# syl051088/DynaAlign

Measured on AMD Instinct MI355X. Metric: sequence-pairs/sec (MinHash k=4 n_hash=500; NW BLOSUM62) at 1/2/4/8 MI355X, higher is better.
Workload: dtype u32

## Files before the change

### dynaalign_amd/csrc/api.cpp

```cpp
#include <sched.h>

#include <algorithm>
#include <atomic>
#include <chrono>
#include <climits>
#include <cmath>
#include <condition_variable>
#include <cstddef>
#include <map>
#include <memory>
#include <cstdlib>
#include <cstring>
#include <functional>
#include <mutex>
#include <random>
#include <string>
#include <thread>
#include <vector>

#include "da_common.hpp"

namespace da { size_t destroy_cached_comms(); }

namespace da {
// ... 326 lines not shown
  return rows;
}
int64_t rows_per_block(int64_t n, size_t bytes_per_elem) { return std::min(block_rows(n, bytes_per_elem), n); }

}
}

using namespace da;

namespace da {
namespace {
bool env_flag(const char *name) { return getenv(name) != nullptr; }
int64_t env_i64(const char *name, int64_t dflt) { const char *e = getenv(name); return e ? atoll(e) : dflt; }
uint64_t env_u64(const char *name, uint64_t dflt) { const char *e = getenv(name); return e ? strtoull(e, nullptr, 10) : dflt; }
enum MhExpand { MH_EXPAND_DEFAULT, MH_EXPAND_ROWS, MH_EXPAND_ROWSPIPE, MH_EXPAND_PIPE, MH_EXPAND_TILES };
Config parse_config() {
  Config c;
  c.mh_no_dedup = env_flag("DYNAALIGN_MH_NO_DEDUP");
  c.mh_no_sparse = env_flag("DYNAALIGN_MH_NO_SPARSE");
  c.mh_no_pipe = env_flag("DYNAALIGN_MH_NO_PIPE");
  c.mh_pipe_one_stream = env_flag("DYNAALIGN_MH_PIPE_ONE_STREAM");
  c.mh_dedup_min_n = env_i64("DYNAALIGN_MH_DEDUP_MIN_N", -1);
  c.mh_dedup_max_pct = env_i64("DYNAALIGN_MH_DEDUP_MAX_PCT", -1);
  c.mh_sparse_max_pairs = std::min<uint64_t>(env_u64("DYNAALIGN_MH_SPARSE_MAX_PAIRS", 400000000ull), 0xfffffff0ull);
  c.mh_no_hybrid = env_flag("DYNAALIGN_MH_NO_HYBRID");
  c.mh_hybrid_min_n = env_i64("DYNAALIGN_MH_HYBRID_MIN_N", -1);
  c.mh_hybrid_dedup = env_flag("DYNAALIGN_MH_HYBRID_DEDUP");
  if (const char *e = getenv("DYNAALIGN_MH_EXPAND"))
    c.mh_expand = !strcmp(e, "rows") ? MH_EXPAND_ROWS : !strcmp(e, "rowspipe") ? MH_EXPAND_ROWSPIPE : !strcmp(e, "pipe") ? MH_EXPAND_PIPE
                : !strcmp(e, "tiles") ? MH_EXPAND_TILES : MH_EXPAND_DEFAULT;
  c.mh_pipe_step = (int)std::max<int64_t>(0, env_i64("DYNAALIGN_MH_PIPE_STEP", 0));
  c.mh_pipe_wg = (int)std::max<int64_t>(0, std::min<int64_t>(4, env_i64("DYNAALIGN_MH_PIPE_WG", 0)));
  c.mh_pipe_head = (int)std::max<int64_t>(0, env_i64("DYNAALIGN_MH_PIPE_HEAD", 0));
  const int pb = (int)env_i64("DYNAALIGN_PLANE_BITS", 0);
  c.plane_bits = (pb == 32 || pb == 16 || pb == 15 || pb == 14 || pb == 12) ? pb : 0;
  c.k2_no_asm = env_flag("DYNAALIGN_K2_NO_ASM");
  c.k2_persist = env_flag("DYNAALIGN_K2_PERSIST");
  c.k2_wg_per_cu = (int)std::max<int64_t>(0, env_i64("DYNAALIGN_K2_WG_PER_CU", 0));
  c.nw_no_dedup = env_flag("DYNAALIGN_NW_NO_DEDUP");
  c.nw_int32 = env_flag("DYNAALIGN_NW_INT32");
  c.nw_no_prefix = env_flag("DYNAALIGN_NW_NO_PREFIX_SHARE");
  c.nw_dedup_min_n = env_i64("DYNAALIGN_NW_DEDUP_MIN_N", -1);
  c.no_host_widen = env_flag("DYNAALIGN_NO_HOST_WIDEN");
  c.plain_d2h = env_flag("DYNAALIGN_PLAIN_D2H");
  c.no_buffer_cache = env_flag("DYNAALIGN_NO_BUFFER_CACHE");
  c.d2h_threads = (int)std::max<int64_t>(0, env_i64("DYNAALIGN_D2H_THREADS", 0));
  c.buffer_cache_pct = (int)std::max<int64_t>(0, std::min<int64_t>(90, env_i64("DYNAALIGN_BUFFER_CACHE_PCT", 30)));
  c.block_bytes = env_u64("DYNAALIGN_BLOCK_BYTES", 0);
  c.trace = env_flag("DYNAALIGN_TRACE");
  c.louvain_debug = env_flag("DYNAALIGN_LOUVAIN_DEBUG");
  c.louvain_threads = (int)std::max<int64_t>(0, env_i64("DYNAALIGN_LOUVAIN_THREADS", 0));
  return c;
}
std::atomic<const Config *> g_config{nullptr};
}
const Config &config() {
  const Config *c = g_config.load(std::memory_order_acquire);
  if (!c) {
    const Config *fresh = new Config(parse_config());
    if (g_config.compare_exchange_strong(c, fresh, std::memory_order_acq_rel)) c = fresh;
    else delete fresh;
  }
  return *c;
}
}
extern "C" void da_config_reload(void) { da::g_config.store(new da::Config(da::parse_config()), std::memory_order_release); }
// ... 371 lines not shown
  const hipStream_t stream = k.stream;
  int rc;
  const bool two = expand_stream_packed(k.n_hash);
  const int wg = cfg.mh_pipe_wg > 0 ? cfg.mh_pipe_wg : two ? 2 : 1, head = cfg.mh_pipe_head > 0 ? cfg.mh_pipe_head : two ? 1 : 4,
            step = cfg.mh_pipe_step > 0 ? cfg.mh_pipe_step : two ? 8 : 4;
  const bool alt = !cfg.mh_pipe_one_stream;
  std::vector<int64_t> cuts{0};
  while (cuts.back() < KB) cuts.push_back(std::min(KB, cuts.back() + (cuts.size() == 1 ? head : step)));
  const size_t C = cuts.size() - 1;
  const PipeLease lease(3 * C + 2);
  PipeRes *const pr = lease.r;
  if (!pr) return MH_NO_PIPE;
  hipEvent_t *pe = pr->ev.data();
  DA_HIP_TRY(hipStreamWaitEvent(pr->side, k.ev[2], 0));
  if ((rc = launch_mh_compare_edges_u16(c.planes.as<uint32_t>(), U, k.n_hash, k.dtab, k.ld_d, stream, c.bits, k.pk)) != DA_OK) return rc;
  if ((rc = launch_expand_stream_lists(k.d.p.uidx, k.n, U, k.ex, stream)) != DA_OK) return rc;
  DA_HIP_TRY(hipEventRecord(pe[3 * C], stream));
  if (c.split()) {
    if ((rc = c.lists(stream)) != DA_OK) return rc;
    DA_HIP_TRY(hipEventRecord(pe[3 * C + 1], stream));
  }
  if (alt) { DA_HIP_TRY(hipStreamWaitEvent(pr->alt[0], pe[3 * C], 0)); DA_HIP_TRY(hipStreamWaitEvent(pr->alt[1], pe[3 * C], 0)); }
  for (size_t ci = 0; ci < C; ++ci) {
    if ((rc = launch_mh_compare_bands_u16(c.planes.as<uint32_t>(), U, k.n_hash, k.dtab, k.ld_d, cuts[ci], cuts[ci + 1], ci == 0 ? 4 : wg, pr->side, c.bits,
                                          k.pk)) != DA_OK) return rc;
    if (c.split()) {
      if (ci == 0) { DA_HIP_TRY(hipStreamWaitEvent(pr->side, pe[3 * C], 0)); DA_HIP_TRY(hipStreamWaitEvent(pr->side, pe[3 * C + 1], 0)); }
      if ((rc = c.fixup(DA_OUT_COMPACT, k.dtab, k.ld_d, pr->side, cuts[ci] * 8, cuts[ci + 1] * 8)) != DA_OK) return rc;
    }
    DA_HIP_TRY(hipEventRecord(pe[3 * ci], pr->side));
    const hipStream_t es = alt ? pr->alt[ci & 1] : stream;
    DA_HIP_TRY(hipStreamWaitEvent(es, pe[3 * ci], 0));
    DA_HIP_TRY(hipEventRecord(pe[3 * ci + 1], es));
    if ((rc = launch_expand_stream_rows(k.dtab, k.ld_d, k.d.p.uidx, k.n, U, k.n_hash, k.out, k.ld, k.ex, cuts[ci] * 1024, cuts[ci + 1] * 1024, es,
                                        (int)ci, k.pk)) != DA_OK) return rc;
    DA_HIP_TRY(hipEventRecord(pe[3 * ci + 2], es));
  }
  if (alt) for (size_t ci = (C >= 2 ? C - 2 : 0); ci < C; ++ci) DA_HIP_TRY(hipStreamWaitEvent(stream, pe[3 * ci + 2], 0));
  if ((rc = mh_finish(k, 5, MH_ROWS_PIPE, 2)) != DA_OK) return rc;
  k.route.chunks = k.route.expand_launches = (int)C;
  MhEvents::ms(k.route, 2, k.ev[2], pe[3 * (C - 1)]);
  MhEvents::ms(k.route, 3, k.ev[2], pe[3 * C]);
  LaunchUnion expand{k.ev[2]};
  for (size_t ci = 0; ci < C; ++ci) expand.add(pe[3 * ci + 1], pe[3 * ci + 2]);
  k.route.ms[4] = expand.total;
  return DA_OK;
}
static int mh_tiles_pipe(const MhCall &k) {
  const Config &cfg = da::config();
  const MhCodes &c = k.c;
  uint16_t *ftab = static_cast<uint16_t *>(k.ex);
  const hipStream_t stream = k.stream;
  const std::vector<int32_t> &ub = k.d.ub;
  const int64_t U = k.d.U, KB = mh_sym_bands(U), NB = (int64_t)ub.size() - 1, ld_f = ceil_div(k.n, 8) * 8;
  int rc;
  const int step = cfg.mh_pipe_step > 0 ? cfg.mh_pipe_step : 4, wg = cfg.mh_pipe_wg > 0 ? cfg.mh_pipe_wg : 2;
  const bool alt = !cfg.mh_pipe_one_stream;
  struct Chunk { int64_t kb0, kb1, ob0, ob1; };
  std::vector<Chunk> chunks;
  for (int64_t kb = 0, ob = 0; kb < KB;) {
    const int64_t kb1 = std::min(KB, kb + (chunks.empty() ? 1 : step));
    int64_t ob1 = ob;
    if (kb1 == KB) ob1 = NB;
    else while (ob1 < NB && (int64_t)ub[(size_t)ob1 + 1] <= kb1 * 1024) ++ob1;
    chunks.push_back({kb, kb1, ob, ob1});
    kb = kb1; ob = ob1;
  }
  const size_t C = chunks.size();
// ... 2941 lines not shown
```

### dynaalign_amd/csrc/da_common.hpp

```cpp
#pragma once

#include <hip/hip_runtime.h>

#include <cstdarg>
#include <cstdint>
#include <cstdio>
#include <string>

#include "../../include/dynaalign.h"

namespace da {
struct Config {
  bool mh_no_dedup = false, mh_no_sparse = false, mh_no_pipe = false, mh_pipe_one_stream = false;
  int64_t mh_dedup_min_n = -1, mh_dedup_max_pct = -1;
  uint64_t mh_sparse_max_pairs = 400000000ull;
  bool mh_no_hybrid = false, mh_hybrid_dedup = false;
  int64_t mh_hybrid_min_n = -1;
  int mh_expand = 0;
  int mh_pipe_step = 0, mh_pipe_wg = 0, mh_pipe_head = 0;
  int plane_bits = 0;
  bool k2_no_asm = false, k2_persist = false;
  int k2_wg_per_cu = 0;
  bool nw_no_dedup = false, nw_int32 = false, nw_no_prefix = false;
  int64_t nw_dedup_min_n = -1;
  bool no_host_widen = false, plain_d2h = false, no_buffer_cache = false;
  int d2h_threads = 0, buffer_cache_pct = 30;
  uint64_t block_bytes = 0;
  bool trace = false, louvain_debug = false;
  int louvain_threads = 0;
};
const Config &config();


std::string &last_error_ref();
int fail(int code, const char *fmt, ...) __attribute__((format(printf, 2, 3)));

#define DA_HIP_TRY(expr)                                                              \
  do {                                                                                \
    hipError_t _e = (expr);                                                           \
    if (_e != hipSuccess)                                                             \
      return ::da::fail(_e == hipErrorNoDevice || _e == hipErrorInvalidDevice         \
                            ? DA_ERR_NO_DEVICE                                        \
                            : DA_ERR_HIP,                                             \
                        "%s failed: %s (%s:%d)", #expr, hipGetErrorString(_e),        \
                        __FILE__, __LINE__);                                          \
  } while (0)

inline int64_t ceil_div(int64_t a, int64_t b) { return (a + b - 1) / b; }
inline int block_shape_ok(int64_t rows, int64_t n) {
  if (rows > 0x7fffffffLL || n > 0x7ffffff0LL) return fail(DA_ERR_UNSUPPORTED, "key block too large for one launch");
  return DA_OK;
}
// ... 120 lines not shown
                   nullptr, nullptr, nullptr, c0, c1);
}
size_t nw_sort_unique_workspace_bytes(int64_t n);
int launch_nw_sort_unique(const uint8_t *d_codes, const int64_t *d_off, int64_t n, void *d_work, size_t work_bytes, const int32_t **perm_out,
                          const uint8_t **lcp_out, hipStream_t stream);
struct NwDedupPlan {
  uint32_t *table; uint32_t table_size;
  int32_t *rep, *mult, *last, *fm, *fs, *pm, *ps, *uid_of, *uidx, *ufirst, *ulast, *ulen, *minfirst, *maxlast;
  int64_t *uoff;
  uint8_t *ucodes;
  size_t bytes;
};
NwDedupPlan nw_dedup_layout(void *work, int64_t n, int64_t total);
size_t nw_dedup_workspace_bytes(int64_t n, int64_t total);
int launch_nw_dedup_count(const uint8_t *d_codes, const int64_t *d_off, int64_t n, const NwDedupPlan &p, hipStream_t stream);
int launch_nw_dedup_build(const uint8_t *d_codes, const int64_t *d_off, int64_t n, int64_t U, const NwDedupPlan &p, hipStream_t stream,
                          bool first_order = false);
int launch_expand_unique(const uint16_t *d_D, int64_t ld_d, const int32_t *d_uidx, int64_t n, int kind, bool is_nw, int n_hash,
                         void *d_out, int64_t ld, hipStream_t stream, int nw_max_len = 0, uint16_t *d_F = nullptr,
                         const int32_t *d_ufirst = nullptr, int64_t U = 0, hipEvent_t after_gather = nullptr, hipEvent_t after_rows = nullptr,
                         int table_world = 1, int64_t table_rows_local = 0,
                         bool only_leftover = false);
bool expand_stream_ok(int64_t n, int64_t U, int n_hash, const void *d_out, int64_t ld);
size_t expand_stream_scratch_bytes(int64_t n, int64_t U);
bool expand_stream_packed(int n_hash);
int launch_expand_stream(const uint16_t *d_D, int64_t ld_d, const int32_t *d_uidx, int64_t n, int64_t U, int n_hash, double *d_out, int64_t ld,
                         void *d_scratch, hipStream_t stream, hipEvent_t after_lists = nullptr, bool pk = false);
int launch_expand_stream_lists(const int32_t *d_uidx, int64_t n, int64_t U, void *d_scratch, hipStream_t stream);
bool expand_stream_rect_ok(int64_t m, int64_t n, int64_t U_x, int64_t U_y, int n_hash, const void *d_out, int64_t ld);
int launch_expand_stream_rect(const uint16_t *d_D, int64_t ld_d, const int32_t *d_uidx_x, int64_t m, int64_t U_x, const int32_t *d_uidx_y, int64_t n,
                              int64_t U_y, int n_hash, double *d_out, int64_t ld, void *d_scratch, hipStream_t stream,
                              hipEvent_t after_lists = nullptr);
int launch_expand_stream_rows(const uint16_t *d_D, int64_t ld_d, const int32_t *d_uidx, int64_t n, int64_t U, int n_hash, double *d_out, int64_t ld,
                              void *d_scratch, int64_t row_begin, int64_t row_end, hipStream_t stream, int launch_no,
                              bool pk = false);
int launch_expand_rows(const uint16_t *d_F, int64_t ld_f, const int32_t *d_uidx, int64_t n, bool is_nw, int n_hash, int nw_max_len,
                       double *d_out, int64_t ld, int64_t band_begin, int64_t band_end, hipStream_t stream);
size_t expand_rows_workspace_bytes(int64_t n, int64_t U, int kind, bool is_nw, int n_hash, int nw_max_len);
int launch_upper_histogram(const uint16_t *d_m, int64_t ld, int64_t n, int nbins, unsigned long long *d_hist,
                           hipStream_t stream, int rank = 0, int world = 0, const int32_t *d_rowmap = nullptr);
int launch_extract_edges(const uint16_t *d_m, int64_t ld, int64_t n, const uint8_t *d_keep, int nbins,
                         bool include_diagonal, int32_t *d_i, int32_t *d_j, uint16_t *d_v, int64_t capacity,
                         unsigned long long *d_count, hipStream_t stream, int rank = 0, int world = 0,
                         const int32_t *d_rowmap = nullptr);
int launch_gather_columns(const uint16_t *d_D, int64_t ld_d, const int32_t *d_uidx, const int32_t *d_ufirst, int64_t n, int64_t U,
                          uint16_t *d_F, int64_t ld_f, bool from_first_tile, hipStream_t stream, int table_world = 1,
                          int64_t table_rows_local = 0, int64_t row_begin = 0, int64_t row_end = -1);
size_t edges_to_csr_workspace_bytes(int64_t m, int64_t n);
int launch_edges_to_csr(const int32_t *d_i, const int32_t *d_j, const uint16_t *d_v, int64_t m, int64_t n, void *d_work, size_t work_bytes,
                        int64_t *d_ptr, int32_t *d_adj, uint16_t *d_codes, uint16_t *d_loops, hipStream_t stream);
size_t knn_edges_workspace_bytes(int64_t n, int top);
int launch_knn_edges(const int32_t *d_idx, const uint16_t *d_key, int64_t ld, int64_t n, int top, bool mutual, bool is_nw, const uint16_t *d_self_key,
                     int self_code, bool loops, void *d_work, size_t work_bytes, int32_t *d_i, int32_t *d_j, uint16_t *d_v, uint64_t *d_count,
                     hipStream_t stream);
constexpr int DA_TOPK_MAX = 1024;
int launch_topk_rows(const uint16_t *d_keys, int64_t rows, int64_t n, int64_t ld, const uint16_t *d_rank, int rank_bits, int top, int32_t *d_idx,
                     int64_t ld_idx, uint16_t *d_key_out, int64_t ld_key, hipStream_t stream);
int launch_topk_rows_self(const uint16_t *d_keys, int64_t rows, int64_t n, int64_t ld, const uint16_t *d_rank, int rank_bits, int top, int64_t self_col0,
                          int32_t *d_idx, int64_t ld_idx, uint16_t *d_key_out, int64_t ld_key, uint16_t *d_self_key, hipStream_t stream);
int launch_topk_ranks(const uint32_t *d_keys, int64_t rows, int64_t n, int64_t ld, int64_t nbins, int top, int32_t *d_idx, int64_t ld_idx,
                      uint32_t *d_key_out, int64_t ld_key, hipStream_t stream);
int launch_topk_ranks_self(const uint32_t *d_keys, int64_t rows, int64_t n, int64_t ld, int64_t nbins, int top, int64_t self_col0, int32_t *d_idx,
                           int64_t ld_idx, uint32_t *d_key_out, int64_t ld_key, uint32_t *d_self_key, hipStream_t stream);
int launch_topk_values(const uint16_t *d_key, int64_t ld_key, int64_t rows, int top, int n_hash, double *d_val, int64_t ld_val, hipStream_t stream);
size_t threshold_rows_workspace_bytes(int64_t rows);
int launch_rect_histogram(const uint16_t *d_keys, int64_t rows, int64_t n, int64_t ld, int nbins, unsigned long long *d_hist, hipStream_t stream);
int launch_threshold_rows_count(const uint16_t *d_keys, int64_t rows, int64_t n, int64_t ld, const uint8_t *d_keep, int nbins, int64_t *d_rowptr,
// ... 37 lines not shown
```

### dynaalign_amd/csrc/minhash_kernels.hip

```cpp
#include "da_common.hpp"

#include <algorithm>
#include <atomic>
#include <mutex>
#include <vector>
#include <type_traits>

namespace da {
namespace {

__device__ __forceinline__ uint32_t rotl32(uint32_t v, int r) {
  return __builtin_rotateleft32(v, r);
}
__device__ __forceinline__ uint32_t mm3_scramble(uint32_t w) {
  w *= 0xcc9e2d51u;
  w = rotl32(w, 15);
  w *= 0x1b873593u;
  return w;
}
__device__ __forceinline__ uint32_t mm3_mix(uint32_t h, uint32_t kk) {
  h ^= kk;
  return rotl32(h, 13) * 5u + 0xe6546b64u;
}
__device__ __forceinline__ uint32_t mm3_final(uint32_t h, uint32_t len) {
// ... 1620 lines not shown
  double *tab = reinterpret_cast<double *>(er_lds + 128 * ER_STRIDE);
  const int64_t L = tile_begin + (int64_t)(blockIdx.x & 7) * per_xcd + (blockIdx.x >> 3);
  if (L >= ntiles || L >= tile_begin + (int64_t)((blockIdx.x & 7) + 1) * per_xcd) return;
  const TileId tt = decode_tile(L, T128, T128, true);
  if (!tt.valid || !expand_fast_takes(tt.ti, tt.tj, n, ld, out)) return;
  const int tid = threadIdx.x, wave = tid >> 6, lane = tid & 63;
  const int tx = ((wave & 1) << 3) + (lane & 7), ty = ((wave >> 1) << 3) + (lane >> 3);
  const int64_t I0 = (int64_t)tt.ti * 128, J0 = (int64_t)tt.tj * 128;
  uint4 st[8];
#pragma unroll
  for (int q = 0; q < 8; ++q) {
    const int row = (tid >> 4) + 16 * q;
    st[q] = *(reinterpret_cast<const uint4 *>(F + (int64_t)uidx[I0 + row] * ld_f + J0) + (tid & 15));
  }
  if (IS_NW) {
    for (int e = tid; e < tab_entries; e += 256) {
      const int mt = e / tab_stride, ln = e - mt * tab_stride;
      tab[e] = ln == 0 ? __longlong_as_double(0xFFF8000000000000ULL) : (double)mt / (double)ln;
    }
  } else {
    for (int e = tid; e < tab_entries; e += 256) tab[e] = (double)e / (double)n_hash;
  }
#pragma unroll
  for (int q = 0; q < 8; ++q)
    *reinterpret_cast<uint4 *>(er_lds + ((tid >> 4) + 16 * q) * ER_STRIDE + (tid & 15) * 16) = st[q];
  __syncthreads();
  auto widen = [&](uint32_t x) -> double {
    if (IS_NW) return tab[(x >> 8) * (uint32_t)tab_stride + (x & 255u)];
    return tab[x];
  };
  er_store_tile(er_lds, widen, out, ld, I0, J0, tx, ty);
}

constexpr int ES_THREADS = 1024, ES_COPIES = 4, ES_TICKETS = 128;
__global__ __launch_bounds__(256) void k_es_count(const int32_t *__restrict__ uidx, int n, uint32_t *__restrict__ cnt) {
  const int i = blockIdx.x * 256 + threadIdx.x;
  if (i < n) atomicAdd(&cnt[uidx[i]], 1u);
}
__global__ __launch_bounds__(1024) void k_es_scan(const uint32_t *__restrict__ cnt, int U, uint32_t *__restrict__ cstart, uint32_t *__restrict__ istart) {
  __shared__ uint64_t wsum[16];
  __shared__ uint64_t carry_s;
  const int tid = threadIdx.x, lane = tid & 63, wave = tid >> 6;
  if (tid == 0) carry_s = 0;
  __syncthreads();
  for (int base = 0; base < U; base += 1024) {
    const int u = base + tid;
    const uint32_t c = u < U ? cnt[u] : 0u;
    const uint64_t v = (uint64_t)c | ((uint64_t)((c + ES_COPIES - 1) / ES_COPIES) << 32);
    uint64_t x = v;
#pragma unroll
    for (int d = 1; d < 64; d <<= 1) {
      const uint64_t y = __shfl_up(x, d, 64);
      if (lane >= d) x += y;
    }
    if (lane == 63) wsum[wave] = x;
    __syncthreads();
    uint64_t woff = 0;
    for (int w = 0; w < wave; ++w) woff += wsum[w];
    const uint64_t carry = carry_s;
    if (u < U) {
      const uint64_t e = carry + woff + x - v;
      cstart[u] = (uint32_t)e;
      istart[u] = (uint32_t)(e >> 32);
    }
    __syncthreads();
    if (tid == 1023) carry_s = carry + woff + x;
    __syncthreads();
  }
  if (tid == 0) { cstart[U] = (uint32_t)carry_s; istart[U] = (uint32_t)(carry_s >> 32); }
}
__global__ __launch_bounds__(256) void k_es_fill(const int32_t *__restrict__ uidx, int n, int U, const uint32_t *__restrict__ cstart,
                                                 const uint32_t *__restrict__ istart, uint32_t *__restrict__ cursor, int32_t *__restrict__ cpos,
                                                 int2 *__restrict__ items) {
  const int i = blockIdx.x * 256 + threadIdx.x;
  if (i < n) {
    const int u = uidx[i];
    cpos[cstart[u] + atomicAdd(&cursor[u], 1u)] = i;
  }
  if (i < U) {
    const uint32_t first = istart[i], cnt = istart[i + 1] - first;
    for (uint32_t q = 0; q < cnt; ++q) items[first + q] = make_int2(i, (int)(q * ES_COPIES));
  }
}
__device__ __forceinline__ double es_ratio(uint32_t c, double dn, double rcp) {
  const double dc = (double)c, q0 = __dmul_rn(dc, rcp), e = __fma_rn(-q0, dn, dc);
  return __fma_rn(e, rcp, q0);
}
__global__ __launch_bounds__(256) void k_es_ratio_check(int n_hash, double *__restrict__ out) {
  const int c = blockIdx.x * 256 + threadIdx.x;
  const double dn = (double)n_hash, rcp = 1.0 / dn;
  if (c <= n_hash) out[c] = es_ratio((uint32_t)c, dn, rcp);
}
enum { ES_U16 = 0, ES_U16_PK = 1, ES_PK = 2 };
template <int FMT, int NQ>
__global__ __launch_bounds__(ES_THREADS, 8)
void k_expand_stream(const uint16_t *__restrict__ D, int64_t ld_d, const int32_t *__restrict__ uidx,
                                                              const uint32_t *__restrict__ cstart, const int32_t *__restrict__ cpos,
                                                              const int2 *__restrict__ items, const uint32_t *__restrict__ istart, int row_begin,
                                                              int row_end, int n, int n_hash, double *__restrict__ out, int64_t ld,
                                                              uint32_t *__restrict__ ticket) {
  extern __shared__ __attribute__((aligned(16))) unsigned char es_lds[];
#ifdef ES_PRIO
  __builtin_amdgcn_s_setprio(ES_PRIO);
#endif
  constexpr bool PACKED = FMT != ES_U16;
  uint16_t *row = reinterpret_cast<uint16_t *>(es_lds);
  unsigned char *row_lo = es_lds, *row_hi = row_lo + ld_d;
  const int tid = threadIdx.x;
  const double dn = (double)n_hash, rcp = 1.0 / dn;
  auto count_of = [&](int c) -> uint32_t {
    if (!PACKED) return row[c];
    return (uint32_t)row_lo[c] | ((((uint32_t)row_hi[c >> 3] >> (c & 7)) & 1u) << 8);
  };
  const int n_items = (int)istart[row_end];
  const int64_t row_bytes = FMT == ES_PK ? pk_row_bytes(ld_d) : 2 * ld_d;
  const int units = (int)(row_bytes >> 4);
  uint4 pre[NQ];
#define ES_FETCH(r_)                                                                                    \
  {                                                                                                     \
    const uint4 *src_ = reinterpret_cast<const uint4 *>(reinterpret_cast<const unsigned char *>(D) + (int64_t)(r_) * row_bytes); \
    _Pragma("unroll") for (int q = 0; q < NQ; ++q) {                                                    \
      const int u = tid + q * ES_THREADS;                                                               \
      pre[q] = u < units ? src_[u] : make_uint4(0, 0, 0, 0);                                            \
    }                                                                                                   \
  }
  __shared__ int s_next;
  const int base = (int)istart[row_begin];
  int k = base + (int)blockIdx.x;
  int2 it = k < n_items ? items[k] : make_int2(0, 0);
  if (k < n_items) ES_FETCH(it.x)
  const int2 *u2 = reinterpret_cast<const int2 *>(uidx);
  const int j2_end = n >> 1;
  while (k < n_items) {
    __syncthreads();
    if (tid == 0) s_next = base + (int)gridDim.x + (int)atomicAdd(ticket, 1u);
    uint4 *dst = reinterpret_cast<uint4 *>(row);
#pragma unroll
    for (int q = 0; q < NQ; ++q) {
      const int u = tid + q * ES_THREADS;
      if (u >= units) continue;
      if (FMT != ES_U16_PK) { dst[u] = pre[q]; continue; }
      const uint4 v = pre[q];
      uint2 lo;
      lo.x = __builtin_amdgcn_perm(v.y, v.x, 0x06040200u);
      lo.y = __builtin_amdgcn_perm(v.w, v.z, 0x06040200u);
      *reinterpret_cast<uint2 *>(row_lo + 8 * u) = lo;
      row_hi[u] = (unsigned char)(((v.x >> 8) & 1u) | ((v.x >> 23) & 2u) | ((v.y >> 6) & 4u) | ((v.y >> 21) & 8u) | ((v.z >> 4) & 16u) |
                                  ((v.z >> 19) & 32u) | ((v.w >> 2) & 64u) | ((v.w >> 17) & 128u));
    }
    __syncthreads();
    const uint32_t c0 = cstart[it.x] + (uint32_t)it.y, c_end = cstart[it.x + 1];
    const int ncop = (int)min((uint32_t)ES_COPIES, c_end - c0);
    double *orow[ES_COPIES];
#pragma unroll
    for (int q = 0; q < ES_COPIES; ++q) orow[q] = out + (int64_t)cpos[c0 + (uint32_t)min(q, ncop - 1)] * ld;
    const int kn = __builtin_amdgcn_readfirstlane(s_next);
    int2 itn = make_int2(0, 0);
    if (kn < n_items) { itn = items[kn]; ES_FETCH(itn.x) }
#pragma unroll 4
    for (int j2 = tid; j2 < j2_end; j2 += ES_THREADS) {
      const int2 c = u2[j2];
      const double v0 = es_ratio(count_of(c.x), dn, rcp), v1 = es_ratio(count_of(c.y), dn, rcp);
      nt_store2(orow[0] + 2 * j2, v0, v1);
      if (ncop > 1) nt_store2(orow[1] + 2 * j2, v0, v1);
      if (ncop > 2) nt_store2(orow[2] + 2 * j2, v0, v1);
      if (ncop > 3) nt_store2(orow[3] + 2 * j2, v0, v1);
    }
    if ((n & 1) && tid == 0) {
      const double v = es_ratio(count_of(uidx[n - 1]), dn, rcp);
      for (int q = 0; q < ncop; ++q) orow[q][n - 1] = v;
    }
    it = itn;
    k = kn;
  }
#undef ES_FETCH
}

bool expand_stream_ok(int64_t n, int64_t U, int n_hash, const void *d_out, int64_t ld) {
  return n >= 2 && n <= 0x7fffffffLL && U >= 1 && U <= 65536 && n_hash >= 1 && n_hash <= 2047 && (ld & 1) == 0 &&
         (reinterpret_cast<uintptr_t>(d_out) & 15) == 0;
}
extern "C" int da_debug_ratio_check(int n_hash, double *d_out, void *stream) {
  if (n_hash < 1 || !d_out) return fail(DA_ERR_BAD_ARG, "ratio check: bad arguments");
  hipLaunchKernelGGL(k_es_ratio_check, dim3((unsigned)(n_hash / 256 + 1)), dim3(256), 0, static_cast<hipStream_t>(stream), n_hash, d_out);
  DA_HIP_TRY(hipGetLastError());
  return DA_OK;
}
bool expand_stream_packed(int n_hash) { return n_hash <= 511; }
size_t expand_stream_scratch_bytes(int64_t n, int64_t U) {
  return ((size_t)(4 * U + 8 + ES_TICKETS) * 4 + (size_t)n * 4 + (size_t)(U + n / ES_COPIES + 2) * 8 + 1024);
}
struct EsLists { uint32_t *cnt, *cursor, *ticket, *cstart, *istart; int32_t *cpos; int2 *items; };
static EsLists es_layout(void *d_scratch, int64_t n, int64_t U) {
  uint32_t *w = static_cast<uint32_t *>(d_scratch);
  EsLists L;
  L.cnt = w; L.cursor = w + U; L.ticket = w + 2 * U; L.cstart = L.ticket + ES_TICKETS; L.istart = L.cstart + (U + 1);
  L.cpos = reinterpret_cast<int32_t *>(L.istart + (U + 1));
  L.items = reinterpret_cast<int2 *>((reinterpret_cast<uintptr_t>(L.cpos + n) + 15) & ~(uintptr_t)15);
  return L;
}
int launch_expand_stream_lists(const int32_t *d_uidx, int64_t n, int64_t U, void *d_scratch, hipStream_t stream) {
  const EsLists L = es_layout(d_scratch, n, U);
  DA_HIP_TRY(hipMemsetAsync(L.cnt, 0, ((size_t)U * 2 + ES_TICKETS) * 4, stream));
  const unsigned nb = (unsigned)ceil_div(std::max(n, U), 256);
  hipLaunchKernelGGL(k_es_count, dim3((unsigned)ceil_div(n, 256)), dim3(256), 0, stream, d_uidx, (int)n, L.cnt);
  hipLaunchKernelGGL(k_es_scan, dim3(1), dim3(1024), 0, stream, L.cnt, (int)U, L.cstart, L.istart);
  hipLaunchKernelGGL(k_es_fill, dim3(nb), dim3(256), 0, stream, d_uidx, (int)n, (int)U, L.cstart, L.istart, L.cursor, L.cpos, L.items);
  DA_HIP_TRY(hipGetLastError());
  return DA_OK;
}
static int es_launch(const uint16_t *d_D, int64_t ld_d, const int32_t *d_colids, int64_t n_cols, const EsLists &L, int64_t n_rows, int64_t row_begin,
                     int64_t row_end, int n_hash, double *d_out, int64_t ld, hipStream_t stream, int launch_no, bool pk);
int launch_expand_stream_rows(const uint16_t *d_D, int64_t ld_d, const int32_t *d_uidx, int64_t n, int64_t U, int n_hash, double *d_out, int64_t ld,
                              void *d_scratch, int64_t row_begin, int64_t row_end, hipStream_t stream, int launch_no, bool pk) {
  if (!expand_stream_ok(n, U, n_hash, d_out, ld) || (ld_d & (pk ? 127 : 7)) || ld_d > 65536 || (reinterpret_cast<uintptr_t>(d_D) & 15) || launch_no < 0 ||
      launch_no >= ES_TICKETS || (pk && !expand_stream_packed(n_hash)))
    return fail(DA_ERR_UNSUPPORTED, "row expansion: shape not covered");
  if (row_end > U) row_end = U;
  if (row_begin >= row_end) return DA_OK;
  return es_launch(d_D, ld_d, d_uidx, n, es_layout(d_scratch, n, U), n, row_begin, row_end, n_hash, d_out, ld, stream, launch_no, pk);
}
static int es_launch(const uint16_t *d_D, int64_t ld_d, const int32_t *d_uidx, int64_t n, const EsLists &L, int64_t n_rows, int64_t row_begin,
                     int64_t row_end, int n_hash, double *d_out, int64_t ld, hipStream_t stream, int launch_no, bool pk) {
  static std::atomic<int> es_cus;
  static std::atomic<uint64_t> es_attr_done;
  int dev = 0;
  DA_HIP_TRY(hipGetDevice(&dev));
  if (!((es_attr_done.load() >> (dev & 63)) & 1u)) {
    hipDeviceProp_t prop;
    DA_HIP_TRY(hipGetDeviceProperties(&prop, dev));
#define DA_ES_ATTR(P, Q) DA_HIP_TRY(hipFuncSetAttribute(reinterpret_cast<const void *>(k_expand_stream<P, Q>), hipFuncAttributeMaxDynamicSharedMemorySize, 65536 * 2))
    DA_ES_ATTR(ES_U16, 2); DA_ES_ATTR(ES_U16, 4); DA_ES_ATTR(ES_U16, 6); DA_ES_ATTR(ES_U16, 8);
    DA_ES_ATTR(ES_U16_PK, 2); DA_ES_ATTR(ES_U16_PK, 4); DA_ES_ATTR(ES_U16_PK, 6); DA_ES_ATTR(ES_U16_PK, 8);
    DA_ES_ATTR(ES_PK, 2); DA_ES_ATTR(ES_PK, 4); DA_ES_ATTR(ES_PK, 6); DA_ES_ATTR(ES_PK, 8);
#undef DA_ES_ATTR
    es_cus.store(prop.multiProcessorCount > 0 ? prop.multiProcessorCount : 256);
    es_attr_done.fetch_or(1ull << (dev & 63));
  }
  const bool packed = pk || expand_stream_packed(n_hash);
  size_t lds = packed ? (size_t)pk_row_bytes(ld_d) : (size_t)ld_d * 2;
  lds = std::max<size_t>(lds, 82 * 1024);
  int64_t grid = (int64_t)es_cus.load();
  grid = std::min<int64_t>(grid, (row_end - row_begin) + n_rows / ES_COPIES + 1);
#define DA_ES(P, Q) hipLaunchKernelGGL((k_expand_stream<P, Q>), dim3((unsigned)grid), dim3(ES_THREADS), lds, stream, d_D, ld_d, d_uidx, L.cstart, L.cpos, L.items, \
                                       L.istart, (int)row_begin, (int)row_end, (int)n, n_hash, d_out, ld, L.ticket + launch_no)
  const int64_t nq = ceil_div((pk ? pk_row_bytes(ld_d) : 2 * ld_d) >> 4, ES_THREADS);
#define DA_ES_NQ(F) do { if (nq <= 2) DA_ES(F, 2); else if (nq <= 4) DA_ES(F, 4); else if (nq <= 6) DA_ES(F, 6); else DA_ES(F, 8); } while (0)
  if (pk) DA_ES_NQ(ES_PK);
  else if (packed) DA_ES_NQ(ES_U16_PK);
  else DA_ES_NQ(ES_U16);
#undef DA_ES_NQ
#undef DA_ES
  DA_HIP_TRY(hipGetLastError());
  return DA_OK;
}
int launch_expand_stream(const uint16_t *d_D, int64_t ld_d, const int32_t *d_uidx, int64_t n, int64_t U, int n_hash, double *d_out, int64_t ld,
                         void *d_scratch, hipStream_t stream, hipEvent_t after_lists, bool pk) {
  if (!expand_stream_ok(n, U, n_hash, d_out, ld)) return fail(DA_ERR_UNSUPPORTED, "row expansion: shape not covered");
  int rc = launch_expand_stream_lists(d_uidx, n, U, d_scratch, stream);
  if (rc != DA_OK) return rc;
  if (after_lists) DA_HIP_TRY(hipEventRecord(after_lists, stream));
  return launch_expand_stream_rows(d_D, ld_d, d_uidx, n, U, n_hash, d_out, ld, d_scratch, 0, U, stream, 0, pk);
}

bool expand_stream_rect_ok(int64_t m, int64_t n, int64_t U_x, int64_t U_y, int n_hash, const void *d_out, int64_t ld) {
  return m >= 1 && m <= 0x7ffffff0LL && n >= 1 && n <= 0x7ffffff0LL && U_x >= 1 && U_x <= m && U_y >= 1 && U_y <= 65536 && n_hash >= 1 &&
         n_hash <= 2047 && (ld & 1) == 0 && (reinterpret_cast<uintptr_t>(d_out) & 15) == 0;
}
int launch_expand_stream_rect(const uint16_t *d_D, int64_t ld_d, const int32_t *d_uidx_x, int64_t m, int64_t U_x, const int32_t *d_uidx_y, int64_t n,
                              int64_t U_y, int n_hash, double *d_out, int64_t ld, void *d_scratch, hipStream_t stream, hipEvent_t after_lists) {
  if (!expand_stream_rect_ok(m, n, U_x, U_y, n_hash, d_out, ld) || ld_d < U_y || (ld_d & 7) || ld_d > 65536 || (reinterpret_cast<uintptr_t>(d_D) & 15))
    return fail(DA_ERR_UNSUPPORTED, "rectangular row expansion: shape not covered");
  int rc = launch_expand_stream_lists(d_uidx_x, m, U_x, d_scratch, stream);
  if (rc != DA_OK) return rc;
  if (after_lists) DA_HIP_TRY(hipEventRecord(after_lists, stream));
  return es_launch(d_D, ld_d, d_uidx_y, n, es_layout(d_scratch, m, U_x), m, 0, U_x, n_hash, d_out, ld, stream, 0, false);
}

__global__ __launch_bounds__(256) void k_fill_sig_rows(uint32_t *__restrict__ sig, int64_t ld_sig, int64_t m, int64_t m_pad, int n_hash) {
  const int64_t r = m + blockIdx.x;
  if (r >= m_pad) return;
  const uint32_t *src = sig + ((r - m) % m) * ld_sig;
  for (int h = threadIdx.x; h < n_hash; h += 256) sig[r * ld_sig + h] = src[h];
}
int launch_fill_sig_rows(uint32_t *d_sig, int64_t ld_sig, int64_t m, int64_t m_pad, int n_hash, hipStream_t stream) {
  if (m_pad <= m || m <= 0) return DA_OK;
  hipLaunchKernelGGL(k_fill_sig_rows, dim3((unsigned)(m_pad - m)), dim3(256), 0, stream, d_sig, ld_sig, m, m_pad, n_hash);
  DA_HIP_TRY(hipGetLastError());
  return DA_OK;
}

size_t expand_rows_workspace_bytes(int64_t n, int64_t U, int kind, bool is_nw, int n_hash, int nw_max_len) {
  if (kind != DA_OUT_F64 || n < 256 || U > 65536 || U < 1) return 0;
  if (is_nw ? (nw_max_len < 1 || (int64_t)(nw_max_len + 1) * (2 * nw_max_len + 1) > 2048) : (n_hash < 1 || n_hash + 1 > 2048)) return 0;
  return (size_t)U * (size_t)(ceil_div(n, 8) * 8) * 2;
}

int launch_gather_columns(const uint16_t *d_D, int64_t ld_d, const int32_t *d_uidx, const int32_t *d_ufirst, int64_t n, int64_t U,
                          uint16_t *d_F, int64_t ld_f, bool from_first_tile, hipStream_t stream, int table_world, int64_t table_rows_local,
                          int64_t row_begin, int64_t row_end) {
  if (row_end < 0 || row_end > U) row_end = U;
  if (row_begin < 0) row_begin = 0;
  if (U >= 1 && row_begin >= row_end) return DA_OK;
  if (U < 1 || U > 65536 || (ld_d & 7) || ld_d > 65536 || (reinterpret_cast<uintptr_t>(d_D) & 15) || (ld_f & 1))
    return fail(DA_ERR_UNSUPPORTED, "column gather: at most 65536 unique strings, 16-byte aligned table rows");
  const TableRows trows{table_world, table_rows_local};
  const size_t row_bytes = (size_t)ld_d * 2;
  static std::atomic<int> gc_cus;
  static std::atomic<uint64_t> gc_attr_done;
// ... 611 lines not shown
```

Measured before the change: 316.5 billion.

## Partition expand-stream work into XCC-local zones with batched ticket stealing

Splits the row-expansion work lists into eight zones by output row range, each with its own ticket counter. Workgroups read their XCC id to pick a home zone, claim items in batches, and steal from other zones once their own runs out. The aim is less contention on a single global atomic and output writes that stay local to each chiplet. The single-block prefix scan is replaced by a three-kernel multi-block scan so it can handle the larger zone-by-unique key space. The trade-offs are bigger scratch buffers, extra launches, and possibly uneven load across zones.

```diff
diff --git a/dynaalign_amd/csrc/api.cpp b/dynaalign_amd/csrc/api.cpp
--- a/dynaalign_amd/csrc/api.cpp
+++ b/dynaalign_amd/csrc/api.cpp
@@ -382,6 +382,7 @@
   c.mh_pipe_step = (int)std::max<int64_t>(0, env_i64("DYNAALIGN_MH_PIPE_STEP", 0));
   c.mh_pipe_wg = (int)std::max<int64_t>(0, std::min<int64_t>(4, env_i64("DYNAALIGN_MH_PIPE_WG", 0)));
   c.mh_pipe_head = (int)std::max<int64_t>(0, env_i64("DYNAALIGN_MH_PIPE_HEAD", 0));
+  c.mh_expand_zones = (int)env_i64("DYNAALIGN_MH_EXPAND_ZONES", 0);
   const int pb = (int)env_i64("DYNAALIGN_PLANE_BITS", 0);
   c.plane_bits = (pb == 32 || pb == 16 || pb == 15 || pb == 14 || pb == 12) ? pb : 0;
   c.k2_no_asm = env_flag("DYNAALIGN_K2_NO_ASM");
@@ -819,8 +820,7 @@
     const hipStream_t es = alt ? pr->alt[ci & 1] : stream;
     DA_HIP_TRY(hipStreamWaitEvent(es, pe[3 * ci], 0));
     DA_HIP_TRY(hipEventRecord(pe[3 * ci + 1], es));
-    if ((rc = launch_expand_stream_rows(k.dtab, k.ld_d, k.d.p.uidx, k.n, U, k.n_hash, k.out, k.ld, k.ex, cuts[ci] * 1024, cuts[ci + 1] * 1024, es,
-                                        (int)ci, k.pk)) != DA_OK) return rc;
+    if ((rc = launch_expand_stream_rows(k.dtab, k.ld_d, k.d.p.uidx, k.n, U, k.n_hash, k.out, k.ld, k.ex, cuts[ci + 1] * 1024, es, k.pk)) != DA_OK) return rc;
     DA_HIP_TRY(hipEventRecord(pe[3 * ci + 2], es));
   }
   if (alt) for (size_t ci = (C >= 2 ? C - 2 : 0); ci < C; ++ci) DA_HIP_TRY(hipStreamWaitEvent(stream, pe[3 * ci + 2], 0));
diff --git a/dynaalign_amd/csrc/da_common.hpp b/dynaalign_amd/csrc/da_common.hpp
--- a/dynaalign_amd/csrc/da_common.hpp
+++ b/dynaalign_amd/csrc/da_common.hpp
@@ -18,6 +18,7 @@
   int64_t mh_hybrid_min_n = -1;
   int mh_expand = 0;
   int mh_pipe_step = 0, mh_pipe_wg = 0, mh_pipe_head = 0;
+  int mh_expand_zones = 0;
   int plane_bits = 0;
   bool k2_no_asm = false, k2_persist = false;
   int k2_wg_per_cu = 0;
@@ -204,7 +205,7 @@
                               int64_t U_y, int n_hash, double *d_out, int64_t ld, void *d_scratch, hipStream_t stream,
                               hipEvent_t after_lists = nullptr);
 int launch_expand_stream_rows(const uint16_t *d_D, int64_t ld_d, const int32_t *d_uidx, int64_t n, int64_t U, int n_hash, double *d_out, int64_t ld,
-                              void *d_scratch, int64_t row_begin, int64_t row_end, hipStream_t stream, int launch_no,
+                              void *d_scratch, int64_t row_end, hipStream_t stream,
                               bool pk = false);
 int launch_expand_rows(const uint16_t *d_F, int64_t ld_f, const int32_t *d_uidx, int64_t n, bool is_nw, int n_hash, int nw_max_len,
                        double *d_out, int64_t ld, int64_t band_begin, int64_t band_end, hipStream_t stream);
diff --git a/dynaalign_amd/csrc/minhash_kernels.hip b/dynaalign_amd/csrc/minhash_kernels.hip
--- a/dynaalign_amd/csrc/minhash_kernels.hip
+++ b/dynaalign_amd/csrc/minhash_kernels.hip
@@ -1676,21 +1676,37 @@
   er_store_tile(er_lds, widen, out, ld, I0, J0, tx, ty);
 }
 
-constexpr int ES_THREADS = 1024, ES_COPIES = 4, ES_TICKETS = 128;
-__global__ __launch_bounds__(256) void k_es_count(const int32_t *__restrict__ uidx, int n, uint32_t *__restrict__ cnt) {
+constexpr int ES_THREADS = 1024, ES_COPIES = 4, ES_ZONES = 8, ES_BATCH = 16;
+__global__ __launch_bounds__(256) void k_es_zero(uint32_t *__restrict__ w, int words) {
   const int i = blockIdx.x * 256 + threadIdx.x;
-  if (i < n) atomicAdd(&cnt[uidx[i]], 1u);
-}
-__global__ __launch_bounds__(1024) void k_es_scan(const uint32_t *__restrict__ cnt, int U, uint32_t *__restrict__ cstart, uint32_t *__restrict__ istart) {
+  if (i < words) w[i] = 0u;
+}
+__global__ __launch_bounds__(256) void k_es_count(const int32_t *__restrict__ uidx, int n, int U, int Z, uint32_t *__restrict__ cnt) {
+  const int i = blockIdx.x * 256 + threadIdx.x;
+  if (i < n) atomicAdd(&cnt[(i / Z) * U + uidx[i]], 1u);
+}
+__device__ __forceinline__ uint64_t es_scan_load(const uint32_t *__restrict__ cnt, int K, int i) {
+  const uint32_t c = i < K ? cnt[i] : 0u;
+  return (uint64_t)c | ((uint64_t)((c + ES_COPIES - 1) / ES_COPIES) << 32);
+}
+__global__ __launch_bounds__(1024) void k_es_scan_sums(const uint32_t *__restrict__ cnt, int K, uint64_t *__restrict__ bsum) {
+  __shared__ uint64_t wsum[16];
+  uint64_t x = es_scan_load(cnt, K, blockIdx.x * 1024 + threadIdx.x);
+#pragma unroll
+  for (int d = 32; d >= 1; d >>= 1) x += __shfl_xor(x, d, 64);
+  if ((threadIdx.x & 63) == 0) wsum[threadIdx.x >> 6] = x;
+  __syncthreads();
+  if (threadIdx.x == 0) { uint64_t t = 0; for (int w = 0; w < 16; ++w) t += wsum[w]; bsum[blockIdx.x] = t; }
+}
+__global__ __launch_bounds__(1024) void k_es_scan_offsets(uint64_t *__restrict__ bsum, int nblocks) {
   __shared__ uint64_t wsum[16];
   __shared__ uint64_t carry_s;
   const int tid = threadIdx.x, lane = tid & 63, wave = tid >> 6;
   if (tid == 0) carry_s = 0;
   __syncthreads();
-  for (int base = 0; base < U; base += 1024) {
-    const int u = base + tid;
-    const uint32_t c = u < U ? cnt[u] : 0u;
-    const uint64_t v = (uint64_t)c | ((uint64_t)((c + ES_COPIES - 1) / ES_COPIES) << 32);
+  for (int base = 0; base < nblocks; base += 1024) {
+    const int i = base + tid;
+    const uint64_t v = i < nblocks ? bsum[i] : 0;
     uint64_t x = v;
 #pragma unroll
     for (int d = 1; d < 64; d <<= 1) {
@@ -1702,28 +1718,44 @@
     uint64_t woff = 0;
     for (int w = 0; w < wave; ++w) woff += wsum[w];
     const uint64_t carry = carry_s;
-    if (u < U) {
-      const uint64_t e = carry + woff + x - v;
-      cstart[u] = (uint32_t)e;
-      istart[u] = (uint32_t)(e >> 32);
-    }
+    if (i < nblocks) bsum[i] = carry + woff + x - v;
     __syncthreads();
     if (tid == 1023) carry_s = carry + woff + x;
     __syncthreads();
   }
-  if (tid == 0) { cstart[U] = (uint32_t)carry_s; istart[U] = (uint32_t)(carry_s >> 32); }
-}
-__global__ __launch_bounds__(256) void k_es_fill(const int32_t *__restrict__ uidx, int n, int U, const uint32_t *__restrict__ cstart,
-                                                 const uint32_t *__restrict__ istart, uint32_t *__restrict__ cursor, int32_t *__restrict__ cpos,
+  if (tid == 0) bsum[nblocks] = carry_s;
+}
+__global__ __launch_bounds__(1024) void k_es_scan_apply(const uint32_t *__restrict__ cnt, int K, const uint64_t *__restrict__ bsum,
+                                                        uint32_t *__restrict__ cstart, uint32_t *__restrict__ zstart) {
+  __shared__ uint64_t wsum[16];
+  const int tid = threadIdx.x, lane = tid & 63, wave = tid >> 6;
+  const int i = blockIdx.x * 1024 + tid;
+  const uint64_t v = es_scan_load(cnt, K, i);
+  uint64_t x = v;
+#pragma unroll
+  for (int d = 1; d < 64; d <<= 1) {
+    const uint64_t y = __shfl_up(x, d, 64);
+    if (lane >= d) x += y;
+  }
+  if (lane == 63) wsum[wave] = x;
+  __syncthreads();
+  uint64_t woff = bsum[blockIdx.x];
+  for (int w = 0; w < wave; ++w) woff += wsum[w];
+  const uint64_t e = woff + x - v;
+  if (i < K) { cstart[i] = (uint32_t)e; zstart[i] = (uint32_t)(e >> 32); }
+  if (blockIdx.x == gridDim.x - 1 && tid == 0) { const uint64_t t = bsum[gridDim.x]; cstart[K] = (uint32_t)t; zstart[K] = (uint32_t)(t >> 32); }
+}
+__global__ __launch_bounds__(256) void k_es_fill(const int32_t *__restrict__ uidx, int n, int U, int Z, int K, const uint32_t *__restrict__ cstart,
+                                                 const uint32_t *__restrict__ zstart, uint32_t *__restrict__ cursor, int32_t *__restrict__ cpos,
                                                  int2 *__restrict__ items) {
   const int i = blockIdx.x * 256 + threadIdx.x;
   if (i < n) {
-    const int u = uidx[i];
-    cpos[cstart[u] + atomicAdd(&cursor[u], 1u)] = i;
-  }
-  if (i < U) {
-    const uint32_t first = istart[i], cnt = istart[i + 1] - first;
-    for (uint32_t q = 0; q < cnt; ++q) items[first + q] = make_int2(i, (int)(q * ES_COPIES));
+    const int key = (i / Z) * U + uidx[i];
+    cpos[cstart[key] + atomicAdd(&cursor[key], 1u)] = i;
+  }
+  if (i < K) {
+    const uint32_t first = zstart[i], cnt = zstart[i + 1] - first;
+    for (uint32_t q = 0; q < cnt; ++q) items[first + q] = make_int2(i % U, (int)(q * ES_COPIES));
   }
 }
 __device__ __forceinline__ double es_ratio(uint32_t c, double dn, double rcp) {
@@ -1740,9 +1772,9 @@
 __global__ __launch_bounds__(ES_THREADS, 8)
 void k_expand_stream(const uint16_t *__restrict__ D, int64_t ld_d, const int32_t *__restrict__ uidx,
                                                               const uint32_t *__restrict__ cstart, const int32_t *__restrict__ cpos,
-                                                              const int2 *__restrict__ items, const uint32_t *__restrict__ istart, int row_begin,
+                                                              const int2 *__restrict__ items, const uint32_t *__restrict__ zstart, int U, int zones,
                                                               int row_end, int n, int n_hash, double *__restrict__ out, int64_t ld,
-                                                              uint32_t *__restrict__ ticket) {
+                                                              uint32_t *ticket, int max_batch) {
   extern __shared__ __attribute__((aligned(16))) unsigned char es_lds[];
 #ifdef ES_PRIO
   __builtin_amdgcn_s_setprio(ES_PRIO);
@@ -1756,7 +1788,6 @@
     if (!PACKED) return row[c];
     return (uint32_t)row_lo[c] | ((((uint32_t)row_hi[c >> 3] >> (c & 7)) & 1u) << 8);
   };
-  const int n_items = (int)istart[row_end];
   const int64_t row_bytes = FMT == ES_PK ? pk_row_bytes(ld_d) : 2 * ld_d;
   const int units = (int)(row_bytes >> 4);
   uint4 pre[NQ];
@@ -1768,16 +1799,40 @@
       pre[q] = u < units ? src_[u] : make_uint4(0, 0, 0, 0);                                            \
     }                                                                                                   \
   }
-  __shared__ int s_next;
-  const int base = (int)istart[row_begin];
-  int k = base + (int)blockIdx.x;
-  int2 it = k < n_items ? items[k] : make_int2(0, 0);
-  if (k < n_items) ES_FETCH(it.x)
+  __shared__ int s_next, s_end, s_zone;
+  unsigned home;
+  asm volatile("s_getreg_b32 %0, hwreg(HW_REG_XCC_ID)" : "=s"(home));
+  home = (home & 7u) % (unsigned)zones;
+  const uint32_t home_z0 = zstart[home * U], home_lim = zstart[home * U + row_end] - home_z0,
+                 home_all = zstart[home * U + U] - home_z0;
+  const uint32_t share = max(1u, gridDim.x / (unsigned)zones);
+  auto take = [&]() {
+    int tz = -1, tk = 0, te = 0;
+    for (int t = 0; t < zones && tz < 0; ++t) {
+      const int z = (int)((home + (unsigned)t) % (unsigned)zones);
+      const uint32_t z0 = t ? zstart[z * U] : home_z0, lim = t ? zstart[z * U + row_end] - z0 : home_lim,
+                     all = t ? zstart[z * U + U] - z0 : home_all;
+      uint32_t cur = __hip_atomic_load(&ticket[z], __ATOMIC_RELAXED, __HIP_MEMORY_SCOPE_AGENT);
+      while (cur < lim) {
+        const uint32_t b = min(min((uint32_t)max_batch, lim - cur), max(1u, (all - cur) / share));
+        const uint32_t old = atomicCAS(&ticket[z], cur, cur + b);
+        if (old == cur) { tz = z; tk = (int)(z0 + cur); te = tk + (int)b; break; }
+        cur = old;
+      }
+    }
+    s_zone = tz; s_next = tk; s_end = te;
+  };
+  if (tid == 0) take();
+  __syncthreads();
+  int z = __builtin_amdgcn_readfirstlane(s_zone), k = __builtin_amdgcn_readfirstlane(s_next), k_end = __builtin_amdgcn_readfirstlane(s_end);
+  int2 it = z >= 0 ? items[k] : make_int2(0, 0);
+  if (z >= 0) ES_FETCH(it.x)
   const int2 *u2 = reinterpret_cast<const int2 *>(uidx);
   const int j2_end = n >> 1;
-  while (k < n_items) {
+  while (z >= 0) {
     __syncthreads();
-    if (tid == 0) s_next = base + (int)gridDim.x + (int)atomicAdd(ticket, 1u);
+    const bool more = k + 1 < k_end;
+    if (tid == 0 && !more) take();
     uint4 *dst = reinterpret_cast<uint4 *>(row);
 #pragma unroll
     for (int q = 0; q < NQ; ++q) {
@@ -1793,14 +1848,16 @@
                                   ((v.z >> 19) & 32u) | ((v.w >> 2) & 64u) | ((v.w >> 17) & 128u));
     }
     __syncthreads();
-    const uint32_t c0 = cstart[it.x] + (uint32_t)it.y, c_end = cstart[it.x + 1];
+    const int key = z * U + it.x;
+    const uint32_t c0 = cstart[key] + (uint32_t)it.y, c_end = cstart[key + 1];
     const int ncop = (int)min((uint32_t)ES_COPIES, c_end - c0);
     double *orow[ES_COPIES];
 #pragma unroll
     for (int q = 0; q < ES_COPIES; ++q) orow[q] = out + (int64_t)cpos[c0 + (uint32_t)min(q, ncop - 1)] * ld;
-    const int kn = __builtin_amdgcn_readfirstlane(s_next);
+    const int zn = more ? z : __builtin_amdgcn_readfirstlane(s_zone), kn = more ? k + 1 : __builtin_amdgcn_readfirstlane(s_next);
+    if (!more) k_end = __builtin_amdgcn_readfirstlane(s_end);
     int2 itn = make_int2(0, 0);
-    if (kn < n_items) { itn = items[kn]; ES_FETCH(itn.x) }
+    if (zn >= 0) { itn = items[kn]; ES_FETCH(itn.x) }
 #pragma unroll 4
     for (int j2 = tid; j2 < j2_end; j2 += ES_THREADS) {
       const int2 c = u2[j2];
@@ -1815,6 +1872,7 @@
       for (int q = 0; q < ncop; ++q) orow[q][n - 1] = v;
     }
     it = itn;
+    z = zn;
     k = kn;
   }
 #undef ES_FETCH
@@ -1831,41 +1889,68 @@
   return DA_OK;
 }
 bool expand_stream_packed(int n_hash) { return n_hash <= 511; }
-size_t expand_stream_scratch_bytes(int64_t n, int64_t U) {
-  return ((size_t)(4 * U + 8 + ES_TICKETS) * 4 + (size_t)n * 4 + (size_t)(U + n / ES_COPIES + 2) * 8 + 1024);
-}
-struct EsLists { uint32_t *cnt, *cursor, *ticket, *cstart, *istart; int32_t *cpos; int2 *items; };
-static EsLists es_layout(void *d_scratch, int64_t n, int64_t U) {
+static int es_zones() { return config().mh_expand_zones == 1 ? 1 : ES_ZONES; }
+struct EsLists { uint32_t *cnt, *cursor, *ticket, *cstart, *zstart; int32_t *cpos; int2 *items; uint64_t *bsum; int zones, Z, K; size_t bytes; };
+static EsLists es_layout(void *d_scratch, int64_t n, int64_t U, int zones) {
   uint32_t *w = static_cast<uint32_t *>(d_scratch);
   EsLists L;
-  L.cnt = w; L.cursor = w + U; L.ticket = w + 2 * U; L.cstart = L.ticket + ES_TICKETS; L.istart = L.cstart + (U + 1);
-  L.cpos = reinterpret_cast<int32_t *>(L.istart + (U + 1));
+  const int64_t K = (int64_t)zones * U;
+  L.zones = zones; L.Z = (int)ceil_div(n, zones); L.K = (int)K;
+  L.cnt = w; L.cursor = w + K; L.ticket = w + 2 * K; L.cstart = L.ticket + ES_ZONES; L.zstart = L.cstart + (K + 1);
+  L.cpos = reinterpret_cast<int32_t *>(L.zstart + (K + 1));
   L.items = reinterpret_cast<int2 *>((reinterpret_cast<uintptr_t>(L.cpos + n) + 15) & ~(uintptr_t)15);
+  L.bsum = reinterpret_cast<uint64_t *>(L.items + (std::min(n, K) + n / ES_COPIES + 2));
+  L.bytes = (size_t)(reinterpret_cast<unsigned char *>(L.bsum + (ceil_div(K, 1024) + 1)) - static_cast<unsigned char *>(d_scratch));
   return L;
 }
-int launch_expand_stream_lists(const int32_t *d_uidx, int64_t n, int64_t U, void *d_scratch, hipStream_t stream) {
-  const EsLists L = es_layout(d_scratch, n, U);
-  DA_HIP_TRY(hipMemsetAsync(L.cnt, 0, ((size_t)U * 2 + ES_TICKETS) * 4, stream));
-  const unsigned nb = (unsigned)ceil_div(std::max(n, U), 256);
-  hipLaunchKernelGGL(k_es_count, dim3((unsigned)ceil_div(n, 256)), dim3(256), 0, stream, d_uidx, (int)n, L.cnt);
-  hipLaunchKernelGGL(k_es_scan, dim3(1), dim3(1024), 0, stream, L.cnt, (int)U, L.cstart, L.istart);
-  hipLaunchKernelGGL(k_es_fill, dim3(nb), dim3(256), 0, stream, d_uidx, (int)n, (int)U, L.cstart, L.istart, L.cursor, L.cpos, L.items);
+size_t expand_stream_scratch_bytes(int64_t n, int64_t U) {
+  return es_layout(nullptr, n, U, ES_ZONES).bytes + 16;
+}
+static int es_lists(const int32_t *d_uidx, int64_t n, int64_t U, void *d_scratch, int zones, hipStream_t stream) {
+  const EsLists L = es_layout(d_scratch, n, U, zones);
+  const int zero_words = 2 * L.K + ES_ZONES;
+  hipLaunchKernelGGL(k_es_zero, dim3((unsigned)ceil_div(zero_words, 256)), dim3(256), 0, stream, L.cnt, zero_words);
+  const unsigned nblk = (unsigned)ceil_div(L.K, 1024);
+  hipLaunchKernelGGL(k_es_count, dim3((unsigned)ceil_div(n, 256)), dim3(256), 0, stream, d_uidx, (int)n, (int)U, L.Z, L.cnt);
+  hipLaunchKernelGGL(k_es_scan_sums, dim3(nblk), dim3(1024), 0, stream, L.cnt, L.K, L.bsum);
+  hipLaunchKernelGGL(k_es_scan_offsets, dim3(1), dim3(1024), 0, stream, L.bsum, (int)nblk);
+  hipLaunchKernelGGL(k_es_scan_apply, dim3(nblk), dim3(1024), 0, stream, L.cnt, L.K, L.bsum, L.cstart, L.zstart);
+  hipLaunchKernelGGL(k_es_fill, dim3((unsigned)ceil_div(std::max<int64_t>(n, L.K), 256)), dim3(256), 0, stream, d_uidx, (int)n, (int)U, L.Z, L.K,
+                     L.cstart, L.zstart, L.cursor, L.cpos, L.items);
   DA_HIP_TRY(hipGetLastError());
   return DA_OK;
 }
-static int es_launch(const uint16_t *d_D, int64_t ld_d, const int32_t *d_colids, int64_t n_cols, const EsLists &L, int64_t n_rows, int64_t row_begin,
-                     int64_t row_end, int n_hash, double *d_out, int64_t ld, hipStream_t stream, int launch_no, bool pk);
+int launch_expand_stream_lists(const int32_t *d_uidx, int64_t n, int64_t U, void *d_scratch, hipStream_t stream) {
+  return es_lists(d_uidx, n, U, d_scratch, es_zones(), stream);
+}
+extern "C" int da_debug_expand_lists(const int32_t *d_uidx, int64_t n, int64_t U, int zones, void *d_scratch, size_t scratch_bytes, int64_t *offsets_out,
+                                     int *zones_out, void *stream) {
+  if (zones == 0) zones = es_zones();
+  if (n < 1 || n > 0x7fffffffLL || U < 1 || U > 65536 || U > n || (zones != 1 && zones != ES_ZONES) || !offsets_out)
+    return fail(DA_ERR_BAD_ARG, "expand lists: bad arguments");
+  const EsLists L = es_layout(d_scratch, n, U, zones);
+  const unsigned char *b = static_cast<const unsigned char *>(d_scratch);
+  offsets_out[0] = reinterpret_cast<const unsigned char *>(L.cstart) - b; offsets_out[1] = reinterpret_cast<const unsigned char *>(L.zstart) - b;
+  offsets_out[2] = reinterpret_cast<const unsigned char *>(L.cpos) - b; offsets_out[3] = reinterpret_cast<const unsigned char *>(L.items) - b;
+  offsets_out[4] = (int64_t)expand_stream_scratch_bytes(n, U); offsets_out[5] = L.Z;
+  if (zones_out) *zones_out = zones;
+  if (!d_scratch) return DA_OK;
+  if (!d_uidx || scratch_bytes < (size_t)offsets_out[4] || (reinterpret_cast<uintptr_t>(d_scratch) & 15)) return fail(DA_ERR_BAD_ARG, "expand lists: bad scratch");
+  return es_lists(d_uidx, n, U, d_scratch, zones, static_cast<hipStream_t>(stream));
+}
+static int es_launch(const uint16_t *d_D, int64_t ld_d, const int32_t *d_colids, int64_t n_cols, const EsLists &L, int64_t n_rows, int64_t U,
+                     int64_t row_end, int n_hash, double *d_out, int64_t ld, hipStream_t stream, bool pk);
 int launch_expand_stream_rows(const uint16_t *d_D, int64_t ld_d, const int32_t *d_uidx, int64_t n, int64_t U, int n_hash, double *d_out, int64_t ld,
-                              void *d_scratch, int64_t row_begin, int64_t row_end, hipStream_t stream, int launch_no, bool pk) {
-  if (!expand_stream_ok(n, U, n_hash, d_out, ld) || (ld_d & (pk ? 127 : 7)) || ld_d > 65536 || (reinterpret_cast<uintptr_t>(d_D) & 15) || launch_no < 0 ||
-      launch_no >= ES_TICKETS || (pk && !expand_stream_packed(n_hash)))
+                              void *d_scratch, int64_t row_end, hipStream_t stream, bool pk) {
+  if (!expand_stream_ok(n, U, n_hash, d_out, ld) || (ld_d & (pk ? 127 : 7)) || ld_d > 65536 || (reinterpret_cast<uintptr_t>(d_D) & 15) ||
+      (pk && !expand_stream_packed(n_hash)))
     return fail(DA_ERR_UNSUPPORTED, "row expansion: shape not covered");
   if (row_end > U) row_end = U;
-  if (row_begin >= row_end) return DA_OK;
-  return es_launch(d_D, ld_d, d_uidx, n, es_layout(d_scratch, n, U), n, row_begin, row_end, n_hash, d_out, ld, stream, launch_no, pk);
-}
-static int es_launch(const uint16_t *d_D, int64_t ld_d, const int32_t *d_uidx, int64_t n, const EsLists &L, int64_t n_rows, int64_t row_begin,
-                     int64_t row_end, int n_hash, double *d_out, int64_t ld, hipStream_t stream, int launch_no, bool pk) {
+  if (row_end <= 0) return DA_OK;
+  return es_launch(d_D, ld_d, d_uidx, n, es_layout(d_scratch, n, U, es_zones()), n, U, row_end, n_hash, d_out, ld, stream, pk);
+}
+static int es_launch(const uint16_t *d_D, int64_t ld_d, const int32_t *d_uidx, int64_t n, const EsLists &L, int64_t n_rows, int64_t U,
+                     int64_t row_end, int n_hash, double *d_out, int64_t ld, hipStream_t stream, bool pk) {
   static std::atomic<int> es_cus;
   static std::atomic<uint64_t> es_attr_done;
   int dev = 0;
@@ -1885,9 +1970,9 @@
   size_t lds = packed ? (size_t)pk_row_bytes(ld_d) : (size_t)ld_d * 2;
   lds = std::max<size_t>(lds, 82 * 1024);
   int64_t grid = (int64_t)es_cus.load();
-  grid = std::min<int64_t>(grid, (row_end - row_begin) + n_rows / ES_COPIES + 1);
+  grid = std::min<int64_t>(grid, std::min<int64_t>(n_rows, L.K) + n_rows / ES_COPIES + 1);
 #define DA_ES(P, Q) hipLaunchKernelGGL((k_expand_stream<P, Q>), dim3((unsigned)grid), dim3(ES_THREADS), lds, stream, d_D, ld_d, d_uidx, L.cstart, L.cpos, L.items, \
-                                       L.istart, (int)row_begin, (int)row_end, (int)n, n_hash, d_out, ld, L.ticket + launch_no)
+                                       L.zstart, (int)U, L.zones, (int)row_end, (int)n, n_hash, d_out, ld, L.ticket, ES_BATCH * ES_ZONES / L.zones)
   const int64_t nq = ceil_div((pk ? pk_row_bytes(ld_d) : 2 * ld_d) >> 4, ES_THREADS);
 #define DA_ES_NQ(F) do { if (nq <= 2) DA_ES(F, 2); else if (nq <= 4) DA_ES(F, 4); else if (nq <= 6) DA_ES(F, 6); else DA_ES(F, 8); } while (0)
   if (pk) DA_ES_NQ(ES_PK);
@@ -1904,7 +1989,7 @@
   int rc = launch_expand_stream_lists(d_uidx, n, U, d_scratch, stream);
   if (rc != DA_OK) return rc;
   if (after_lists) DA_HIP_TRY(hipEventRecord(after_lists, stream));
-  return launch_expand_stream_rows(d_D, ld_d, d_uidx, n, U, n_hash, d_out, ld, d_scratch, 0, U, stream, 0, pk);
+  return launch_expand_stream_rows(d_D, ld_d, d_uidx, n, U, n_hash, d_out, ld, d_scratch, U, stream, pk);
 }
 
 bool expand_stream_rect_ok(int64_t m, int64_t n, int64_t U_x, int64_t U_y, int n_hash, const void *d_out, int64_t ld) {
@@ -1918,7 +2003,7 @@
   int rc = launch_expand_stream_lists(d_uidx_x, m, U_x, d_scratch, stream);
   if (rc != DA_OK) return rc;
   if (after_lists) DA_HIP_TRY(hipEventRecord(after_lists, stream));
-  return es_launch(d_D, ld_d, d_uidx_y, n, es_layout(d_scratch, m, U_x), m, 0, U_x, n_hash, d_out, ld, stream, 0, false);
+  return es_launch(d_D, ld_d, d_uidx_y, n, es_layout(d_scratch, m, U_x, es_zones()), m, U_x, U_x, n_hash, d_out, ld, stream, false);
 }
 
 __global__ __launch_bounds__(256) void k_fill_sig_rows(uint32_t *__restrict__ sig, int64_t ld_sig, int64_t m, int64_t m_pad, int n_hash) {
```

Result: faster. 322.4 billion (median of 6 runs) (+1.9%).
